# ruc-aimc-lab/GeoFormer

Hardware: AMD Instinct MI355X
Metric: image-pairs/sec (640x640) (higher is better)
Workload: dtype f16

## Files before the change

geoformer_amd/csrc/k3_linear.hip:

```cpp
#include <math.h>

#include <type_traits>

#include "gf_common.h"

#ifndef K3_TRACE
#define K3_TRACE 0
#endif
#if K3_TRACE
__device__ long long k3_trace[1024 * 4 * 16];
#define K3_T(slot) do { if (lane == 0 && blockIdx.y == 0 && blockIdx.x < 1024) k3_trace[(blockIdx.x * 4 + wave) * 16 + (slot)] = clock64(); } while (0)
extern "C" int gf_debug_k3_trace(long long* out) {
    return (int)hipMemcpyFromSymbol(out, HIP_SYMBOL(k3_trace), sizeof(long long) * 1024 * 4 * 16);
}
#else
#define K3_T(slot)
#endif

namespace {

enum { EPI_NONE = 0, EPI_RELU = 1, EPI_TANH = 2, EPI_LN = 3, EPI_LN_RES = 4, EPI_UPADD = 5 };

struct LinArgs {
    const void* a1;
    const void* a2;
    long lda1, lda2;
    int k1, k2;
    const void* w;
    const float* bias;
    const void* rgbias;
    int rg_rows;
    const float* gamma;
    const float* beta;
    float eps;
    const void* res;
    long ldres;
    const int32_t* flag;
    int flag_rows;
    void* out;
    long ldo;
    int M, N;
    const void* up_lo;
    int up_h, up_w, up_H, up_W, up_n;
    float up_ry, up_rx;
    int rm_w;
    long rm_line, rm_pix;
    const unsigned long long* rows;
    const int32_t* grp_count;
    int grp_stride, grp_rows;
};

__device__ __forceinline__ void lin_tile(int& row_tile, int& col_tile) {
    const int gx = gridDim.x, gy = gridDim.y;
    row_tile = blockIdx.x;
    col_tile = blockIdx.y;
    if (gy > 1 && (gx & 7) == 0) {
        const int id = blockIdx.y * gx + blockIdx.x, grp = id / (8 * gy), j = id - grp * (8 * gy);
        row_tile = grp * 8 + (j & 7);
        col_tile = j >> 3;
    }
}

template <typename T, int NB, int EPI, bool CONVX = false, bool AROWS = false>
__global__ __launch_bounds__(256, sizeof(T) == 2 ? 2 : 1) void linear_kernel(LinArgs a) {
    using Mm = Mma32<T>;
    using Frag = typename Mm::Frag;
    constexpr int EPC = 16 / sizeof(T);
    constexpr int BK = 128 / sizeof(T);
    constexpr int WROWS = 32 * NB;
    constexpr int ROWS = 128 + WROWS;
    constexpr int NLD = ROWS * 8 / 256;
    extern __shared__ __attribute__((aligned(16))) char smem[];
    char* st = smem;
    char* sw = smem + 128 * 128;
    float* vec = reinterpret_cast<float*>(smem + ROWS * 128);
    const int tid = threadIdx.x, lane = tid & 63, wave = tid >> 6, h = lane >> 5, lr = lane & 31;
    int row_tile, col_tile;
    lin_tile(row_tile, col_tile);
    const int m0 = row_tile * 128, n0 = col_tile * WROWS;
    const int K = a.k1 + a.k2;
    if constexpr (AROWS) {
        if (a.grp_count) {
            bool needed = false;
            const int mend = min(m0 + 128, a.M);
            for (int g = m0 / a.grp_rows, r = m0; r < mend && !needed; r = ++g * a.grp_rows)
                needed = r - g * a.grp_rows < a.grp_count[(size_t)g * a.grp_stride];
            if (!needed) return;
        }
    }

    if (tid < WROWS) {
        vec[tid] = (a.bias && n0 + tid < a.N) ? a.bias[n0 + tid] : 0.f;
        if constexpr (EPI == EPI_LN || EPI == EPI_LN_RES) {
            vec[WROWS + tid] = a.gamma[n0 + tid];
            vec[2 * WROWS + tid] = a.beta[n0 + tid];
        }
    }
    const T* src[NLD];
    int dst[NLD];
    bool isa[NLD];
#pragma unroll
    for (int p = 0; p < NLD; ++p) {
        const int e = p * 256 + tid, row = e >> 3, c = e & 7;
        isa[p] = row < 128;
        if (isa[p]) {
            src[p] = nullptr;
            if constexpr (AROWS) src[p] = reinterpret_cast<const T*>(a.rows[min(m0 + row, a.M - 1)]);
            dst[p] = gf_lds_off(row, c);
        } else {
            const int wr = row - 128;
            src[p] = (const T*)a.w + (size_t)min(n0 + wr, a.N - 1) * K + c * EPC;
            dst[p] = 128 * 128 + gf_lds_off(wr, c);
        }
    }
    v4u regs[NLD];
    const bool ragged = CONVX && (K % BK) != 0;
    auto gload = [&](int k0) {
        const bool first = k0 < a.k1;
        const T* ab = (const T*)(first ? a.a1 : a.a2);
        const long ld = first ? a.lda1 : a.lda2;
        const int kk = first ? k0 : k0 - a.k1;
#pragma unroll
        for (int p = 0; p < NLD; ++p) {
            const int e = p * 256 + tid, row = e >> 3, c = e & 7;
            const T* g;
            if (isa[p]) {
                if constexpr (AROWS) {
                    g = src[p] + k0 + c * EPC;
                } else {
                    const int r = min(m0 + row, a.M - 1);
                    const size_t ro = (CONVX && a.rm_w > 0) ? (size_t)(r / a.rm_w) * a.rm_line + (size_t)(r % a.rm_w) * a.rm_pix : (size_t)r * ld;
                    g = ab + ro + kk + c * EPC;
                }
            } else {
                g = src[p] + k0;
            }
            if constexpr (AROWS) {
                if (isa[p] && src[p] == nullptr) {
                    regs[p] = v4u{0u, 0u, 0u, 0u};
                    continue;
                }
            }
            if (!ragged || k0 + c * EPC < K) regs[p] = *reinterpret_cast<const v4u*>(g);
            else regs[p] = v4u{0u, 0u, 0u, 0u};
        }
    };
    auto lstore = [&]() {
#pragma unroll
        for (int p = 0; p < NLD; ++p) *reinterpret_cast<v4u*>(smem + dst[p]) = regs[p];
    };
    v16f acc[NB];
#pragma unroll
    for (int nb = 0; nb < NB; ++nb)
#pragma unroll
        for (int r = 0; r < 16; ++r) acc[nb][r] = 0.f;

    const int nk = (K + BK - 1) / BK;
    K3_T(0);
    gload(0);
    for (int kt = 0; kt < nk; ++kt) {
        __syncthreads();
        lstore();
        __syncthreads();
        K3_T(1 + kt);
        if (kt + 1 < nk) gload((kt + 1) * BK);
#pragma unroll
        for (int g = 0; g < 4; ++g) {
            const int chunk = 2 * g + h;
            const Frag tf = *reinterpret_cast<const Frag*>(st + gf_lds_off(wave * 32 + lr, chunk));
#pragma unroll
            for (int nb = 0; nb < NB; ++nb) {
                const Frag wf = *reinterpret_cast<const Frag*>(sw + gf_lds_off(nb * 32 + lr, chunk));
                Mm::mma(wf, tf, acc[nb]);
            }
        }
    }
    K3_T(10);
    const int token = m0 + wave * 32 + lr;
    const bool live = token < a.M;
    const int tk = live ? token : a.M - 1;
#pragma unroll
    for (int nb = 0; nb < NB; ++nb)
#pragma unroll
        for (int r = 0; r < 16; ++r) acc[nb][r] += vec[nb * 32 + gf_acc_row(r, h)];
    if (a.rgbias) {
        const T* rb = (const T*)a.rgbias + (size_t)(tk / a.rg_rows) * a.N + n0;
#pragma unroll
        for (int nb = 0; nb < NB; ++nb)
#pragma unroll
            for (int r = 0; r < 16; ++r) acc[nb][r] += gf_to_float(rb[nb * 32 + gf_acc_row(r, h)]);
    }
    if constexpr (EPI == EPI_RELU) {
#pragma unroll
        for (int nb = 0; nb < NB; ++nb)
#pragma unroll
            for (int r = 0; r < 16; ++r) acc[nb][r] = fmaxf(acc[nb][r], 0.f);
    } else if constexpr (EPI == EPI_TANH) {
#pragma unroll
        for (int nb = 0; nb < NB; ++nb)
#pragma unroll
            for (int r = 0; r < 16; ++r) {
                if constexpr (std::is_same<T, float>::value) acc[nb][r] = tanhf(acc[nb][r]);
                else acc[nb][r] = 1.0f - 2.0f * __builtin_amdgcn_rcpf(__expf(2.0f * acc[nb][r]) + 1.0f);
            }
    } else if constexpr (EPI == EPI_LN || EPI == EPI_LN_RES) {
        float s = 0.f;
#pragma unroll
        for (int nb = 0; nb < NB; ++nb)
#pragma unroll
            for (int r = 0; r < 16; ++r) s += acc[nb][r];
        s += __shfl_xor(s, 32, 64);
        const float mean = s / (float)WROWS;
        float q = 0.f;
#pragma unroll
        for (int nb = 0; nb < NB; ++nb)
#pragma unroll
            for (int r = 0; r < 16; ++r) {
                const float d = acc[nb][r] - mean;
                q += d * d;
            }
        q += __shfl_xor(q, 32, 64);
        const float rstd = 1.0f / sqrtf(q / (float)WROWS + a.eps);
#pragma unroll
        for (int nb = 0; nb < NB; ++nb)
#pragma unroll
            for (int r = 0; r < 16; ++r) {
                const int c = nb * 32 + gf_acc_row(r, h);
                acc[nb][r] = (acc[nb][r] - mean) * rstd * vec[WROWS + c] + vec[2 * WROWS + c];
            }
    }
    if constexpr (!std::is_same<T, float>::value) {
        using V4 = gf_vec<T, 4>;
        using V8 = gf_vec<T, 8>;
        constexpr int RS = 272;
        K3_T(11);
        __syncthreads();
        K3_T(12);
        char* ot = smem + wave * 32 * RS;
        const int prow = lane >> 4, pch = lane & 15;
        int upx = 0, upy = 0, upn = 0;
        if constexpr (EPI == EPI_UPADD) {
            const unsigned t0 = (unsigned)__builtin_amdgcn_readfirstlane(m0 + wave * 32);
            const unsigned q = t0 / (unsigned)a.up_W;
            upx = (int)(t0 - q * (unsigned)a.up_W);
            upy = (int)(q % (unsigned)a.up_H);
            upn = (int)(q / (unsigned)a.up_H);
        }
#pragma unroll
        for (int hb = 0; hb < (NB + 3) / 4; ++hb) {
#pragma unroll
            for (int q4 = 0; q4 < 4; ++q4)
#pragma unroll
                for (int r4 = 0; r4 < 4; ++r4) {
                    const int nb = hb * 4 + q4, c = q4 * 32 + 8 * r4 + 4 * h;
                    if (nb < NB)
                        *reinterpret_cast<V4*>(ot + lr * RS + c * 2) =
                            V4{(T)acc[nb][4 * r4], (T)acc[nb][4 * r4 + 1], (T)acc[nb][4 * r4 + 2], (T)acc[nb][4 * r4 + 3]};
                }
            __builtin_amdgcn_fence(__ATOMIC_RELEASE, "wavefront");
            __builtin_amdgcn_wave_barrier();
            __builtin_amdgcn_fence(__ATOMIC_ACQUIRE, "wavefront");
            if constexpr (EPI == EPI_UPADD) {
                const int cg = n0 + hb * 128 + pch * 8;
                const bool cok = cg < a.N;
                const T* lo = (const T*)a.up_lo + (cok ? cg : 0);
#ifdef K3_EXP_NOGATHER
#define K3_TAP(p) (*reinterpret_cast<const V8*>(lp))
#else
#define K3_TAP(p) (*reinterpret_cast<const V8*>(p))
#endif
#ifndef K3_UPADD_BATCH
#define K3_UPADD_BATCH 4
#endif
                constexpr int UB = K3_UPADD_BATCH;
#pragma unroll
                for (int b0 = 0; b0 < 8; b0 += UB) {
                V8 tap[UB][4];
                float wgt[UB][2];
#pragma unroll
                for (int ib = 0; ib < UB; ++ib) {
                    const int it = b0 + ib;
                    const int row = it * 4 + prow;
                    int px = upx + row, py = upy, pn = upn;
                    if (a.up_W >= 32) {
                        const bool wr = px >= a.up_W;
                        px -= wr ? a.up_W : 0;
                        py += wr ? 1 : 0;
                        const bool wy = py >= a.up_H;
                        py = wy ? 0 : py;
                        pn += wy ? 1 : 0;
                    } else {
                        const unsigned t = (unsigned)(m0 + wave * 32 + row), q = t / (unsigned)a.up_W;
                        px = (int)(t - q * (unsigned)a.up_W);
                        py = (int)(q % (unsigned)a.up_H);
                        pn = (int)(q / (unsigned)a.up_H);
                    }
                    pn = pn < a.up_n ? pn : a.up_n - 1;
                    const float fy = a.up_ry * py, fx = a.up_rx * px;
                    const int y0 = (int)fy, x0 = (int)fx;
                    const int y1 = y0 + (y0 < a.up_h - 1), x1 = x0 + (x0 < a.up_w - 1);
                    wgt[ib][0] = fy - y0;
                    wgt[ib][1] = fx - x0;
                    const T* lp = lo + (size_t)pn * a.up_h * a.up_w * a.N;
                    tap[ib][0] = K3_TAP(lp + ((size_t)y0 * a.up_w + x0) * a.N);
                    tap[ib][1] = K3_TAP(lp + ((size_t)y0 * a.up_w + x1) * a.N);
                    tap[ib][2] = K3_TAP(lp + ((size_t)y1 * a.up_w + x0) * a.N);
                    tap[ib][3] = K3_TAP(lp + ((size_t)y1 * a.up_w + x1) * a.N);
                }
#pragma unroll
                for (int ib = 0; ib < UB; ++ib) {
                    const int row = (b0 + ib) * 4 + prow, tg = m0 + wave * 32 + row;
                    V8 v = *reinterpret_cast<const V8*>(ot + row * RS + pch * 16);
                    const float wy1 = wgt[ib][0], wx1 = wgt[ib][1], wy0 = 1.f - wy1, wx0 = 1.f - wx1;
                    if constexpr (std::is_same<T, _Float16>::value) {
                        const float w00 = wy0 * wx0, w01 = wy0 * wx1, w10 = wy1 * wx0, w11 = wy1 * wx1;
                        const v4u uv = __builtin_bit_cast(v4u, v), u0 = __builtin_bit_cast(v4u, tap[ib][0]), u1 = __builtin_bit_cast(v4u, tap[ib][1]),
                                  u2 = __builtin_bit_cast(v4u, tap[ib][2]), u3 = __builtin_bit_cast(v4u, tap[ib][3]);
#pragma unroll
                        for (int i = 0; i < 4; ++i) {
                            float lo_, hi_;
                            asm("v_fma_mix_f32 %0, %1, %2, %3 op_sel:[0,0,0] op_sel_hi:[1,0,1]" : "=v"(lo_) : "v"(u0[i]), "v"(w00), "v"(uv[i]));
                            asm("v_fma_mix_f32 %0, %1, %2, %3 op_sel:[1,0,1] op_sel_hi:[1,0,1]" : "=v"(hi_) : "v"(u0[i]), "v"(w00), "v"(uv[i]));
                            asm("v_fma_mix_f32 %0, %1, %2, %0 op_sel:[0,0,0] op_sel_hi:[1,0,0]" : "+v"(lo_) : "v"(u1[i]), "v"(w01));
                            asm("v_fma_mix_f32 %0, %1, %2, %0 op_sel:[1,0,0] op_sel_hi:[1,0,0]" : "+v"(hi_) : "v"(u1[i]), "v"(w01));
                            asm("v_fma_mix_f32 %0, %1, %2, %0 op_sel:[0,0,0] op_sel_hi:[1,0,0]" : "+v"(lo_) : "v"(u2[i]), "v"(w10));
                            asm("v_fma_mix_f32 %0, %1, %2, %0 op_sel:[1,0,0] op_sel_hi:[1,0,0]" : "+v"(hi_) : "v"(u2[i]), "v"(w10));
                            asm("v_fma_mix_f32 %0, %1, %2, %0 op_sel:[0,0,0] op_sel_hi:[1,0,0]" : "+v"(lo_) : "v"(u3[i]), "v"(w11));
                            asm("v_fma_mix_f32 %0, %1, %2, %0 op_sel:[1,0,0] op_sel_hi:[1,0,0]" : "+v"(hi_) : "v"(u3[i]), "v"(w11));
                            v[2 * i] = (T)lo_;
                            v[2 * i + 1] = (T)hi_;
                        }
                    } else {
#pragma unroll
                        for (int i = 0; i < 8; ++i)
                            v[i] = (T)((float)v[i] + wy0 * (wx0 * (float)tap[ib][0][i] + wx1 * (float)tap[ib][1][i]) +
                                              wy1 * (wx0 * (float)tap[ib][2][i] + wx1 * (float)tap[ib][3][i]));
                    }
                    if (tg < a.M && cok) *reinterpret_cast<V8*>((T*)a.out + (size_t)tg * a.ldo + cg) = v;
                }
                }
            } else {
#pragma unroll
            for (int it = 0; it < 8; ++it) {
                const int row = it * 4 + prow, tg = m0 + wave * 32 + row, cg = n0 + hb * 128 + pch * 8;
                if (tg >= a.M || cg >= a.N) continue;
                V8 v = *reinterpret_cast<const V8*>(ot + row * RS + pch * 16);
                if constexpr (EPI == EPI_LN_RES) {
                    const V8 x = *reinterpret_cast<const V8*>((const T*)a.res + (size_t)tg * a.ldres + cg);
                    const bool keep = a.flag == nullptr || a.flag[tg / a.flag_rows] != 0;
#pragma unroll
                    for (int i = 0; i < 8; ++i) v[i] = keep ? (T)((float)x[i] + (float)v[i]) : x[i];
                }
                *reinterpret_cast<V8*>((T*)a.out + (size_t)tg * a.ldo + cg) = v;
            }
            }
            __builtin_amdgcn_fence(__ATOMIC_RELEASE, "wavefront");
            __builtin_amdgcn_wave_barrier();
            K3_T(13 + hb);
        }
    } else {
        bool keep = true;
        if constexpr (EPI == EPI_LN_RES) keep = a.flag == nullptr || a.flag[tk / a.flag_rows] != 0;
        if (!live) return;
        T* op = (T*)a.out + (size_t)token * a.ldo + n0;
        const T* rp = EPI == EPI_LN_RES ? (const T*)a.res + (size_t)token * a.ldres + n0 : nullptr;
#pragma unroll
        for (int nb = 0; nb < NB; ++nb)
#pragma unroll
            for (int r4 = 0; r4 < 4; ++r4) {
                const int c = nb * 32 + 8 * r4 + 4 * h;
                if (n0 + c >= a.N) continue;
                v4f v{acc[nb][4 * r4], acc[nb][4 * r4 + 1], acc[nb][4 * r4 + 2], acc[nb][4 * r4 + 3]};
                if constexpr (EPI == EPI_LN_RES) {
                    const v4f x = *reinterpret_cast<const v4f*>(rp + c);
                    v = keep ? v4f{x.x + v.x, x.y + v.y, x.z + v.z, x.w + v.w} : x;
                }
                *reinterpret_cast<v4f*>(op + c) = v;
            }
    }
}

template <typename T, int EPI>
__global__ __launch_bounds__(256, 2) void linear_kernel_w2(LinArgs a) {
    using Frag = typename Mma32<T>::Frag;
    using V4 = gf_vec<T, 4>;
    using V8 = gf_vec<T, 8>;
    constexpr int EPC = 8, BK = 64, WROWS = 256, ROWS = 128 + WROWS, NLD = ROWS * 8 / 256;
    extern __shared__ __attribute__((aligned(16))) char smem[];
    char* st = smem;
    char* sw = smem + 128 * 128;
    float* vec = reinterpret_cast<float*>(smem + ROWS * 128);
    const int tid = threadIdx.x, lane = tid & 63, wave = tid >> 6, h = lane >> 5, lr = lane & 31;
    const int tm = wave >> 1, tn = wave & 1;
    int row_tile, col_tile;
    lin_tile(row_tile, col_tile);
    const int m0 = row_tile * 128, n0 = col_tile * WROWS;
    const int K = a.k1 + a.k2;
    if (tid < WROWS) vec[tid] = (a.bias && n0 + tid < a.N) ? a.bias[n0 + tid] : 0.f;
    const T* src[NLD];
    int dst[NLD];
    bool isa[NLD];
#pragma unroll
    for (int p = 0; p < NLD; ++p) {
        const int e = p * 256 + tid, row = e >> 3, c = e & 7;
        isa[p] = row < 128;
        if (isa[p]) {
            src[p] = nullptr;
            dst[p] = gf_lds_off(row, c);
        } else {
            const int wr = row - 128;
            src[p] = (const T*)a.w + (size_t)min(n0 + wr, a.N - 1) * K + c * EPC;
            dst[p] = 128 * 128 + gf_lds_off(wr, c);
        }
    }
    v4u regs[NLD];
    auto gload = [&](int k0) {
        const bool first = k0 < a.k1;
        const T* ab = (const T*)(first ? a.a1 : a.a2);
        const long ld = first ? a.lda1 : a.lda2;
        const int kk = first ? k0 : k0 - a.k1;
#pragma unroll
        for (int p = 0; p < NLD; ++p) {
            const int e = p * 256 + tid, row = e >> 3, c = e & 7;
            const T* g = isa[p] ? ab + (size_t)min(m0 + row, a.M - 1) * ld + kk + c * EPC : src[p] + k0;
            regs[p] = *reinterpret_cast<const v4u*>(g);
        }
    };
    v16f acc[2][4];
#pragma unroll
    for (int t = 0; t < 2; ++t)
#pragma unroll
        for (int nb = 0; nb < 4; ++nb)
#pragma unroll
            for (int r = 0; r < 16; ++r) acc[t][nb][r] = 0.f;
    const int nk = K / BK;
    gload(0);
    for (int kt = 0; kt < nk; ++kt) {
        __syncthreads();
#pragma unroll
        for (int p = 0; p < NLD; ++p) *reinterpret_cast<v4u*>(smem + dst[p]) = regs[p];
        __syncthreads();
        if (kt + 1 < nk) gload((kt + 1) * BK);
#pragma unroll
        for (int g = 0; g < 4; ++g) {
            const int chunk = 2 * g + h;
            const Frag t0 = *reinterpret_cast<const Frag*>(st + gf_lds_off(tm * 64 + lr, chunk));
            const Frag t1 = *reinterpret_cast<const Frag*>(st + gf_lds_off(tm * 64 + 32 + lr, chunk));
#pragma unroll
            for (int nb = 0; nb < 4; ++nb) {
                const Frag wf = *reinterpret_cast<const Frag*>(sw + gf_lds_off(tn * 128 + nb * 32 + lr, chunk));
                Mma32<T>::mma(wf, t0, acc[0][nb]);
                Mma32<T>::mma(wf, t1, acc[1][nb]);
            }
        }
    }
#pragma unroll
    for (int t = 0; t < 2; ++t)
#pragma unroll
        for (int nb = 0; nb < 4; ++nb)
#pragma unroll
            for (int r = 0; r < 16; ++r) {
                float v = acc[t][nb][r] + vec[tn * 128 + nb * 32 + gf_acc_row(r, h)];
                if constexpr (EPI == EPI_RELU) v = fmaxf(v, 0.f);
                else if constexpr (EPI == EPI_TANH) v = 1.0f - 2.0f * __builtin_amdgcn_rcpf(__expf(2.0f * v) + 1.0f);
                acc[t][nb][r] = v;
            }
    constexpr int RS = 272;
    __syncthreads();
    char* ot = smem + wave * 32 * RS;
    const int prow = lane >> 4, pch = lane & 15;
#pragma unroll
    for (int t = 0; t < 2; ++t) {
#pragma unroll
        for (int nb = 0; nb < 4; ++nb)
#pragma unroll
            for (int r4 = 0; r4 < 4; ++r4) {
                const int c = nb * 32 + 8 * r4 + 4 * h;
                *reinterpret_cast<V4*>(ot + lr * RS + c * 2) =
                    V4{(T)acc[t][nb][4 * r4], (T)acc[t][nb][4 * r4 + 1], (T)acc[t][nb][4 * r4 + 2], (T)acc[t][nb][4 * r4 + 3]};
            }
        __builtin_amdgcn_fence(__ATOMIC_RELEASE, "wavefront");
        __builtin_amdgcn_wave_barrier();
        __builtin_amdgcn_fence(__ATOMIC_ACQUIRE, "wavefront");
#pragma unroll
        for (int it = 0; it < 8; ++it) {
            const int row = it * 4 + prow, tg = m0 + tm * 64 + t * 32 + row, cg = n0 + tn * 128 + pch * 8;
            if (tg >= a.M || cg >= a.N) continue;
            *reinterpret_cast<V8*>((T*)a.out + (size_t)tg * a.ldo + cg) = *reinterpret_cast<const V8*>(ot + row * RS + pch * 16);
        }
        __builtin_amdgcn_fence(__ATOMIC_RELEASE, "wavefront");
        __builtin_amdgcn_wave_barrier();
    }
}

template <typename T, int NB, int EPI, bool CONVX = false, bool AROWS = false>
void lin_launch1(const LinArgs& a, hipStream_t st) {
    constexpr int WROWS = 32 * NB;
    size_t lds = (size_t)(128 + WROWS) * 128 + 3 * WROWS * sizeof(float);
    if (lds < 4 * 32 * 272) lds = 4 * 32 * 272;
    linear_kernel<T, NB, EPI, CONVX, AROWS><<<dim3((a.M + 127) / 128, (a.N + WROWS - 1) / WROWS), 256, lds, st>>>(a);
}

template <typename T, int NB, bool AROWS = false>
void lin_launch(const LinArgs& a, int epi, hipStream_t st) {
    switch (epi) {
        case EPI_NONE: lin_launch1<T, NB, EPI_NONE, false, AROWS>(a, st); break;
        case EPI_RELU: lin_launch1<T, NB, EPI_RELU, false, AROWS>(a, st); break;
        case EPI_TANH: lin_launch1<T, NB, EPI_TANH, false, AROWS>(a, st); break;
        case EPI_LN: lin_launch1<T, NB, EPI_LN, false, AROWS>(a, st); break;
        default: lin_launch1<T, NB, EPI_LN_RES, false, AROWS>(a, st); break;
    }
}

}

extern "C" int gf_linear(const void* a1, long lda1, int k1, const void* a2, long lda2, int k2, const void* w,
                         const float* bias, const void* rowgroup_bias, int rowgroup_rows, int epilogue,
                         const float* ln_gamma, const float* ln_beta, float ln_eps, const void* residual,
                         long ldres, const int32_t* row_flag, int flag_rows, void* out, long ldo, int dtype, int M,
                         int N, void* stream) {
    GF_CHECK_ARG(a1 && w && out, "null pointer");
    GF_CHECK_ARG(M > 0 && N > 0 && k1 > 0 && k2 >= 0, "bad sizes");
    GF_CHECK_ARG(dtype >= GF_F32 && dtype <= GF_BF16, "bad dtype");
    const int bk = dtype == GF_F32 ? 32 : 64;
    GF_CHECK_ARG(k1 % bk == 0 && k2 % bk == 0, "k1 and k2 must be multiples of 32 (f32) / 64 (f16)");
    GF_CHECK_ARG(k2 == 0 || a2 != nullptr, "a2 missing");
    GF_CHECK_ARG(N % 32 == 0, "N must be a multiple of 32");
    GF_CHECK_ARG(epilogue >= EPI_NONE && epilogue <= EPI_LN_RES, "unknown epilogue");
    GF_CHECK_ARG(rowgroup_bias == nullptr || rowgroup_rows > 0, "rowgroup_rows must be > 0");
    GF_CHECK_ARG(rowgroup_bias == nullptr || N % 128 == 0, "a row-group bias needs N to be a multiple of 128 (whole column tiles)");
    const int es = dtype == GF_F32 ? 4 : 2;
    GF_CHECK_ARG((lda1 * es) % 16 == 0 && (k2 == 0 || (lda2 * es) % 16 == 0), "operand rows must be 16-byte aligned");
    GF_CHECK_ARG((ldo * es) % 16 == 0 && (uintptr_t)out % 16 == 0, "output rows must be 16-byte aligned");
    GF_CHECK_ARG(residual == nullptr || ((ldres * es) % 16 == 0 && (uintptr_t)residual % 16 == 0),
                 "residual rows must be 16-byte aligned");
    if (epilogue >= EPI_LN) {
        GF_CHECK_ARG(ln_gamma && ln_beta, "LayerNorm epilogue needs gamma and beta");
        GF_CHECK_ARG(N == 128 || N == 256, "LayerNorm epilogue is built for N = 128 or 256 (whole rows per wave pair)");
        GF_CHECK_ARG(epilogue != EPI_LN_RES || residual != nullptr, "residual missing");
        GF_CHECK_ARG(row_flag == nullptr || flag_rows > 0, "flag_rows must be > 0");
    }
    LinArgs a{a1, a2, lda1, lda2, k1, k2, w, bias, rowgroup_bias, rowgroup_rows, ln_gamma, ln_beta, ln_eps, residual,
              ldres, row_flag, flag_rows, out, ldo, M, N};
    hipStream_t st = (hipStream_t)stream;
    void* pt = gf_prof_begin("k3_linear", st, (double)es * ((double)M * (k1 + k2) + (double)N * (k1 + k2) + (double)M * N * (residual ? 2.0 : 1.0)));
    const bool wide = (epilogue >= EPI_LN) ? N == 256 : N % 256 == 0;
    if (dtype != GF_F32 && wide && epilogue <= EPI_TANH && rowgroup_bias == nullptr) {
        const size_t lds = (size_t)(128 + 256) * 128 + 256 * sizeof(float);
        const dim3 grid((M + 127) / 128, (N + 255) / 256);
#define GF_W2(T)                                                                   \
    do {                                                                           \
        if (epilogue == EPI_NONE) linear_kernel_w2<T, EPI_NONE><<<grid, 256, lds, st>>>(a);       \
        else if (epilogue == EPI_RELU) linear_kernel_w2<T, EPI_RELU><<<grid, 256, lds, st>>>(a);  \
        else linear_kernel_w2<T, EPI_TANH><<<grid, 256, lds, st>>>(a);                            \
    } while (0)
        if (dtype == GF_F16) GF_W2(_Float16);
        else GF_W2(gf_bf16);
#undef GF_W2
    } else if (dtype == GF_F32) {
        if (wide) lin_launch<float, 8>(a, epilogue, st);
        else lin_launch<float, 4>(a, epilogue, st);
    } else if (dtype == GF_F16) {
        if (wide) lin_launch<_Float16, 8>(a, epilogue, st);
        else lin_launch<_Float16, 4>(a, epilogue, st);
    } else {
        if (wide) lin_launch<gf_bf16, 8>(a, epilogue, st);
        else lin_launch<gf_bf16, 4>(a, epilogue, st);
    }
    gf_prof_end("k3_linear", pt, st);
    GF_CHECK_LAUNCH();
    return GF_OK;
}

extern "C" int gf_linear_rows(const uint64_t* row_table, int row_align, const int32_t* group_count, int group_count_stride, int group_rows,
                              int k, const void* w, const float* bias, const void* rowgroup_bias, int rowgroup_rows, int epilogue,
                              const float* ln_gamma, const float* ln_beta, float ln_eps, const void* residual, long ldres,
                              const int32_t* row_flag, int flag_rows, void* out, long ldo, int dtype, int M, int N, void* stream) {
    GF_CHECK_ARG(row_table && w && out, "null pointer");
    GF_CHECK_ARG(dtype == GF_F16 || dtype == GF_BF16, "built for the 16-bit types (fp32: gf_linear on a gathered copy)");
    GF_CHECK_ARG(M > 0 && N > 0 && k > 0, "bad sizes");
    GF_CHECK_ARG(k % 64 == 0, "k must be a multiple of 64");
    GF_CHECK_ARG(N % 32 == 0, "N must be a multiple of 32");
    GF_CHECK_ARG(epilogue >= EPI_NONE && epilogue <= EPI_LN_RES, "unknown epilogue");
    GF_CHECK_ARG(rowgroup_bias == nullptr || rowgroup_rows > 0, "rowgroup_rows must be > 0");
    GF_CHECK_ARG(rowgroup_bias == nullptr || N % 128 == 0, "a row-group bias needs N to be a multiple of 128 (whole column tiles)");
    GF_CHECK_ARG(row_align > 0 && (row_align & (row_align - 1)) == 0 && row_align % 16 == 0, "operand rows must be 16-byte aligned (row_align: a power of two >= 16)");
    GF_CHECK_ARG((uintptr_t)row_table % 8 == 0, "the row table must be 8-byte aligned");
    GF_CHECK_ARG(group_count == nullptr || (group_rows > 0 && group_count_stride >= 0), "group_rows must be > 0");
    GF_CHECK_ARG((ldo * 2) % 16 == 0 && (uintptr_t)out % 16 == 0, "output rows must be 16-byte aligned");
    GF_CHECK_ARG(residual == nullptr || ((ldres * 2) % 16 == 0 && (uintptr_t)residual % 16 == 0), "residual rows must be 16-byte aligned");
    if (epilogue >= EPI_LN) {
        GF_CHECK_ARG(ln_gamma && ln_beta, "LayerNorm epilogue needs gamma and beta");
        GF_CHECK_ARG(N == 128 || N == 256, "LayerNorm epilogue is built for N = 128 or 256 (whole rows per wave pair)");
        GF_CHECK_ARG(epilogue != EPI_LN_RES || residual != nullptr, "residual missing");
        GF_CHECK_ARG(row_flag == nullptr || flag_rows > 0, "flag_rows must be > 0");
    }
    LinArgs a{nullptr, nullptr, 0, 0, k, 0, w, bias, rowgroup_bias, rowgroup_rows, ln_gamma, ln_beta, ln_eps, residual,
              ldres, row_flag, flag_rows, out, ldo, M, N};
    a.rows = (const unsigned long long*)row_table;
    a.grp_count = group_count; a.grp_stride = group_count_stride; a.grp_rows = group_rows;
    hipStream_t st = (hipStream_t)stream;
    const double rows_moved = group_count ? 0.0 : (double)M;
    void* pt = gf_prof_begin("k3_linear", st, 2.0 * (rows_moved * k + (double)N * k + rows_moved * N * (residual ? 2.0 : 1.0)) + 8.0 * M);
    const bool wide = (epilogue >= EPI_LN) ? N == 256 : N % 256 == 0;
    if (dtype == GF_F16) {
        if (wide) lin_launch<_Float16, 8, true>(a, epilogue, st);
        else lin_launch<_Float16, 4, true>(a, epilogue, st);
    } else {
        if (wide) lin_launch<gf_bf16, 8, true>(a, epilogue, st);
        else lin_launch<gf_bf16, 4, true>(a, epilogue, st);
    }
    gf_prof_end("k3_linear", pt, st);
    GF_CHECK_LAUNCH();
    return GF_OK;
}

namespace {
__global__ __launch_bounds__(256) void index_rows_kernel(const char* x, long row_bytes, const int32_t* idx, long idx_stride, int N, int L,
                                                         unsigned long long* rows) {
    const long e = (long)blockIdx.x * 256 + threadIdx.x;
    if (e >= (long)N * L) return;
    const long n = e / L, j = e - n * L;
    const int t = min(max(idx[n * idx_stride + j], 0), L - 1);
    rows[e] = (unsigned long long)(uintptr_t)(x + (n * L + t) * row_bytes);
}
}

extern "C" int gf_index_rows(const void* x, long row_bytes, const int32_t* idx, long idx_stride, int N, int L, uint64_t* rows, void* stream) {
    GF_CHECK_ARG(x && idx && rows, "null pointer");
    GF_CHECK_ARG(N > 0 && L > 0 && (long)N * L < (1l << 31) && row_bytes > 0 && idx_stride >= 0, "bad sizes");
    index_rows_kernel<<<(unsigned)(((long)N * L + 255) / 256), 256, 0, (hipStream_t)stream>>>((const char*)x, row_bytes, idx, idx_stride, N, L,
                                                                                              (unsigned long long*)rows);
    GF_CHECK_LAUNCH();
    return GF_OK;
}

extern "C" int gf_conv1x1_upsample_add_nhwc(const void* x, const void* w, const void* lo, void* out, int N, int h, int wl,
                                            int H, int W, int Cin, int Cout, int dtype, void* stream) {
    GF_CHECK_ARG(x && w && lo && out, "null pointer");
    GF_CHECK_ARG(N > 0 && h > 0 && wl > 0 && H > 0 && W > 0, "empty problem");
    GF_CHECK_ARG(dtype == GF_F16 || dtype == GF_BF16, "built for 16-bit maps (the inference backbone)");
    GF_CHECK_ARG(Cin % 32 == 0 && Cout % 32 == 0, "Cin and Cout must be multiples of 32");
    GF_CHECK_ARG((long)N * H * W < (1l << 31), "too many pixels");
    GF_CHECK_ARG((uintptr_t)x % 16 == 0 && (uintptr_t)out % 16 == 0 && (uintptr_t)lo % 16 == 0, "tensors must be 16-byte aligned");
    LinArgs a{};
    a.a1 = x; a.lda1 = Cin; a.k1 = Cin; a.w = w; a.out = out; a.ldo = Cout; a.M = N * H * W; a.N = Cout;
    a.up_lo = lo; a.up_h = h; a.up_w = wl; a.up_H = H; a.up_W = W; a.up_n = N;
    a.up_ry = H > 1 ? (float)(h - 1) / (float)(H - 1) : 0.f;
    a.up_rx = W > 1 ? (float)(wl - 1) / (float)(W - 1) : 0.f;
    hipStream_t st = (hipStream_t)stream;
    void* pt = gf_prof_begin("k3_upadd", st, 2.0 * ((double)a.M * (Cin + Cout) + (double)N * h * wl * Cout + (double)Cin * Cout));
    if (dtype == GF_F16) lin_launch1<_Float16, 4, EPI_UPADD, true>(a, st);
    else lin_launch1<gf_bf16, 4, EPI_UPADD, true>(a, st);
    gf_prof_end("k3_upadd", pt, st);
    GF_CHECK_LAUNCH();
    return GF_OK;
}

extern "C" int gf_conv1x1_nhwc(const void* x, const void* w, void* out, int N, int H, int W, int Cin, int Cout, int stride, int dtype,
                               void* stream) {
    GF_CHECK_ARG(x && w && out, "null pointer");
    GF_CHECK_ARG(N > 0 && H > 0 && W > 0, "empty problem");
    GF_CHECK_ARG(stride == 1 || (stride == 2 && H % 2 == 0 && W % 2 == 0), "stride 1, or 2 on even-sized maps");
    GF_CHECK_ARG(dtype == GF_F16 || dtype == GF_BF16, "built for 16-bit maps (the inference backbone)");
    GF_CHECK_ARG(Cin % 32 == 0 && Cout % 32 == 0, "Cin and Cout must be multiples of 32");
    GF_CHECK_ARG((long)N * H * W < (1l << 31), "too many pixels");
    GF_CHECK_ARG((uintptr_t)x % 16 == 0 && (uintptr_t)out % 16 == 0 && (uintptr_t)w % 16 == 0, "tensors must be 16-byte aligned");
    const int oh = H / stride, ow = W / stride;
    LinArgs a{};
    a.a1 = x; a.lda1 = Cin; a.k1 = Cin; a.w = w; a.out = out; a.ldo = Cout; a.M = N * oh * ow; a.N = Cout;
    if (stride == 2) { a.rm_w = ow; a.rm_line = 2l * W * Cin; a.rm_pix = 2l * Cin; }
    hipStream_t st = (hipStream_t)stream;
    void* pt = gf_prof_begin("conv1x1", st, 2.0 * ((double)a.M * (Cin + Cout) + (double)Cin * Cout));
    if (dtype == GF_F16) lin_launch1<_Float16, 4, EPI_NONE, true>(a, st);
    else lin_launch1<gf_bf16, 4, EPI_NONE, true>(a, st);
    gf_prof_end("conv1x1", pt, st);
    GF_CHECK_LAUNCH();
    return GF_OK;
}
```

Measured before the change: 731.2.

## Add persistent streaming GEMM for small-K linears with register-resident weights

Adds a persistent linear_stream kernel for K<=256 that keeps each wave's weight fragment in registers and double-buffers 64-row activation tiles into LDS by DMA. Each block loops over tiles assigned per XCD, so the next tile's load overlaps the current tile's MMA and epilogue. The kernel is routed ahead of the existing paths for linear, conv1x1 and upsample-add calls, and the bilinear blend is factored into a shared helper. In exchange it adds a new code path with 32-bit offset limits and an XCD-based tile split whose load balance and occupancy may differ from the tiled kernels.

```diff
diff --git a/geoformer_amd/csrc/k3_linear.hip b/geoformer_amd/csrc/k3_linear.hip
--- a/geoformer_amd/csrc/k3_linear.hip
+++ b/geoformer_amd/csrc/k3_linear.hip
@@ -58,6 +58,35 @@
         const int id = blockIdx.y * gx + blockIdx.x, grp = id / (8 * gy), j = id - grp * (8 * gy);
         row_tile = grp * 8 + (j & 7);
         col_tile = j >> 3;
+    }
+}
+
+template <typename T>
+__device__ __forceinline__ void k3_upadd_blend(gf_vec<T, 8>& v, const gf_vec<T, 8> (&tap)[4], float wy1, float wx1) {
+    const float wy0 = 1.f - wy1, wx0 = 1.f - wx1;
+    if constexpr (std::is_same<T, _Float16>::value) {
+        const float w00 = wy0 * wx0, w01 = wy0 * wx1, w10 = wy1 * wx0, w11 = wy1 * wx1;
+        const v4u uv = __builtin_bit_cast(v4u, v), u0 = __builtin_bit_cast(v4u, tap[0]), u1 = __builtin_bit_cast(v4u, tap[1]),
+                  u2 = __builtin_bit_cast(v4u, tap[2]), u3 = __builtin_bit_cast(v4u, tap[3]);
+#pragma unroll
+        for (int i = 0; i < 4; ++i) {
+            float lo_, hi_;
+            asm("v_fma_mix_f32 %0, %1, %2, %3 op_sel:[0,0,0] op_sel_hi:[1,0,1]" : "=v"(lo_) : "v"(u0[i]), "v"(w00), "v"(uv[i]));
+            asm("v_fma_mix_f32 %0, %1, %2, %3 op_sel:[1,0,1] op_sel_hi:[1,0,1]" : "=v"(hi_) : "v"(u0[i]), "v"(w00), "v"(uv[i]));
+            asm("v_fma_mix_f32 %0, %1, %2, %0 op_sel:[0,0,0] op_sel_hi:[1,0,0]" : "+v"(lo_) : "v"(u1[i]), "v"(w01));
+            asm("v_fma_mix_f32 %0, %1, %2, %0 op_sel:[1,0,0] op_sel_hi:[1,0,0]" : "+v"(hi_) : "v"(u1[i]), "v"(w01));
+            asm("v_fma_mix_f32 %0, %1, %2, %0 op_sel:[0,0,0] op_sel_hi:[1,0,0]" : "+v"(lo_) : "v"(u2[i]), "v"(w10));
+            asm("v_fma_mix_f32 %0, %1, %2, %0 op_sel:[1,0,0] op_sel_hi:[1,0,0]" : "+v"(hi_) : "v"(u2[i]), "v"(w10));
+            asm("v_fma_mix_f32 %0, %1, %2, %0 op_sel:[0,0,0] op_sel_hi:[1,0,0]" : "+v"(lo_) : "v"(u3[i]), "v"(w11));
+            asm("v_fma_mix_f32 %0, %1, %2, %0 op_sel:[1,0,0] op_sel_hi:[1,0,0]" : "+v"(hi_) : "v"(u3[i]), "v"(w11));
+            v[2 * i] = (T)lo_;
+            v[2 * i + 1] = (T)hi_;
+        }
+    } else {
+#pragma unroll
+        for (int i = 0; i < 8; ++i)
+            v[i] = (T)((float)v[i] + wy0 * (wx0 * (float)tap[0][i] + wx1 * (float)tap[1][i]) +
+                       wy1 * (wx0 * (float)tap[2][i] + wx1 * (float)tap[3][i]));
     }
 }
 
@@ -311,31 +340,7 @@
                 for (int ib = 0; ib < UB; ++ib) {
                     const int row = (b0 + ib) * 4 + prow, tg = m0 + wave * 32 + row;
                     V8 v = *reinterpret_cast<const V8*>(ot + row * RS + pch * 16);
-                    const float wy1 = wgt[ib][0], wx1 = wgt[ib][1], wy0 = 1.f - wy1, wx0 = 1.f - wx1;
-                    if constexpr (std::is_same<T, _Float16>::value) {
-                        const float w00 = wy0 * wx0, w01 = wy0 * wx1, w10 = wy1 * wx0, w11 = wy1 * wx1;
-                        const v4u uv = __builtin_bit_cast(v4u, v), u0 = __builtin_bit_cast(v4u, tap[ib][0]), u1 = __builtin_bit_cast(v4u, tap[ib][1]),
-                                  u2 = __builtin_bit_cast(v4u, tap[ib][2]), u3 = __builtin_bit_cast(v4u, tap[ib][3]);
-#pragma unroll
-                        for (int i = 0; i < 4; ++i) {
-                            float lo_, hi_;
-                            asm("v_fma_mix_f32 %0, %1, %2, %3 op_sel:[0,0,0] op_sel_hi:[1,0,1]" : "=v"(lo_) : "v"(u0[i]), "v"(w00), "v"(uv[i]));
-                            asm("v_fma_mix_f32 %0, %1, %2, %3 op_sel:[1,0,1] op_sel_hi:[1,0,1]" : "=v"(hi_) : "v"(u0[i]), "v"(w00), "v"(uv[i]));
-                            asm("v_fma_mix_f32 %0, %1, %2, %0 op_sel:[0,0,0] op_sel_hi:[1,0,0]" : "+v"(lo_) : "v"(u1[i]), "v"(w01));
-                            asm("v_fma_mix_f32 %0, %1, %2, %0 op_sel:[1,0,0] op_sel_hi:[1,0,0]" : "+v"(hi_) : "v"(u1[i]), "v"(w01));
-                            asm("v_fma_mix_f32 %0, %1, %2, %0 op_sel:[0,0,0] op_sel_hi:[1,0,0]" : "+v"(lo_) : "v"(u2[i]), "v"(w10));
-                            asm("v_fma_mix_f32 %0, %1, %2, %0 op_sel:[1,0,0] op_sel_hi:[1,0,0]" : "+v"(hi_) : "v"(u2[i]), "v"(w10));
-                            asm("v_fma_mix_f32 %0, %1, %2, %0 op_sel:[0,0,0] op_sel_hi:[1,0,0]" : "+v"(lo_) : "v"(u3[i]), "v"(w11));
-                            asm("v_fma_mix_f32 %0, %1, %2, %0 op_sel:[1,0,0] op_sel_hi:[1,0,0]" : "+v"(hi_) : "v"(u3[i]), "v"(w11));
-                            v[2 * i] = (T)lo_;
-                            v[2 * i + 1] = (T)hi_;
-                        }
-                    } else {
-#pragma unroll
-                        for (int i = 0; i < 8; ++i)
-                            v[i] = (T)((float)v[i] + wy0 * (wx0 * (float)tap[ib][0][i] + wx1 * (float)tap[ib][1][i]) +
-                                              wy1 * (wx0 * (float)tap[ib][2][i] + wx1 * (float)tap[ib][3][i]));
-                    }
+                    k3_upadd_blend<T>(v, tap[ib], wgt[ib][0], wgt[ib][1]);
                     if (tg < a.M && cok) *reinterpret_cast<V8*>((T*)a.out + (size_t)tg * a.ldo + cg) = v;
                 }
                 }
@@ -491,6 +496,197 @@
         __builtin_amdgcn_fence(__ATOMIC_RELEASE, "wavefront");
         __builtin_amdgcn_wave_barrier();
     }
+}
+
+constexpr int ST_TM = 64;
+constexpr int ST_OT = ST_TM * 256;
+
+template <typename T, int KG, int EPI>
+__global__ __launch_bounds__(256, 2) void linear_stream(LinArgs a, int tiles, int ncb, unsigned a_bytes) {
+    using Mm = Mma32<T>;
+    using Frag = typename Mm::Frag;
+    using V4 = gf_vec<T, 4>;
+    using V8 = gf_vec<T, 8>;
+    constexpr int RB = KG * 32, CPR = RB / 16, RPP = 64 / CPR, NP = ST_TM / RPP / 4, TILE = ST_TM * RB;
+    extern __shared__ __attribute__((aligned(16))) char smem[];
+    char* ot = smem + 2 * TILE;
+    const int tid = threadIdx.x, lane = tid & 63, wave = __builtin_amdgcn_readfirstlane(tid >> 6), h = lane >> 5, lr = lane & 31;
+    const int xcd = blockIdx.x & 7, slot = blockIdx.x >> 3, per_xcd = gridDim.x >> 3;
+    const int cb = slot % ncb, rl = slot / ncb, nrl = per_xcd / ncb;
+    const int tq = tiles >> 3, trem = tiles & 7;
+    const int tbeg = xcd < trem ? xcd * (tq + 1) : trem * (tq + 1) + (xcd - trem) * tq, tcnt = tq + (xcd < trem ? 1 : 0);
+    if (rl >= tcnt) return;
+    const int K = a.k1, n0 = cb * 128, nw = n0 + wave * 32;
+    Frag af[KG];
+    {
+        const T* wp = (const T*)a.w + (size_t)min(nw + lr, a.N - 1) * K + h * 8;
+#pragma unroll
+        for (int kg = 0; kg < KG; ++kg) {
+            if (kg * 16 < K) af[kg] = *reinterpret_cast<const Frag*>(wp + kg * 16);
+            else af[kg] = __builtin_bit_cast(Frag, v4u{0u, 0u, 0u, 0u});
+        }
+    }
+    float bv[16];
+#pragma unroll
+    for (int r = 0; r < 16; ++r) {
+        const int n = nw + gf_acc_row(r, h);
+        bv[r] = (a.bias && n < a.N) ? a.bias[n] : 0.f;
+    }
+    const GfRsrc ars = gf_rsrc(a.a1, a_bytes);
+    auto dma = [&](int tile, int buf) {
+        int dl = lane;
+        asm volatile("" : "+v"(dl));
+#pragma unroll
+        for (int i = 0; i < NP; ++i) {
+            const int p = wave * NP + i, row = p * RPP + dl / CPR, c = (dl % CPR) ^ (row & 15);
+            const unsigned r = (unsigned)(tile * ST_TM + row);
+            unsigned ro;
+            if (a.rm_w > 0) {
+                const unsigned y = r / (unsigned)a.rm_w;
+                ro = y * (unsigned)a.rm_line + (r - y * (unsigned)a.rm_w) * (unsigned)a.rm_pix;
+            } else {
+                ro = r * (unsigned)a.lda1;
+            }
+            const bool in = r < (unsigned)a.M && c * 8 < K;
+            gf_lds_dma(ars, smem + buf * TILE + p * 1024, in ? (int)((ro + c * 8) * (unsigned)sizeof(T)) : 0x7FFFFFF0, 0);
+        }
+    };
+    dma(tbeg + rl, 0);
+    int it = 0;
+    for (int ti = rl; ti < tcnt; ti += nrl, ++it) {
+        const int tile = tbeg + ti, m0 = tile * ST_TM;
+        asm volatile("s_waitcnt vmcnt(0)" ::: "memory");
+        __syncthreads();
+        if (ti + nrl < tcnt) dma(tile + nrl, (it + 1) & 1);
+        const char* tb = smem + (it & 1) * TILE;
+        v16f acc[2];
+#pragma unroll
+        for (int t = 0; t < 2; ++t)
+#pragma unroll
+            for (int r = 0; r < 16; ++r) acc[t][r] = 0.f;
+#pragma unroll
+        for (int kg = 0; kg < KG; ++kg) {
+            const int chunk = 2 * kg + h;
+            const Frag b0 = *reinterpret_cast<const Frag*>(tb + lr * RB + ((chunk ^ (lr & 15)) << 4));
+            const Frag b1 = *reinterpret_cast<const Frag*>(tb + (32 + lr) * RB + ((chunk ^ (lr & 15)) << 4));
+            Mm::mma(af[kg], b0, acc[0]);
+            Mm::mma(af[kg], b1, acc[1]);
+        }
+#pragma unroll
+        for (int t = 0; t < 2; ++t)
+#pragma unroll
+            for (int r = 0; r < 16; ++r) acc[t][r] += bv[r];
+        if (a.rgbias) {
+#pragma unroll
+            for (int t = 0; t < 2; ++t) {
+                const int tk = min(m0 + t * 32 + lr, a.M - 1);
+                const T* rb = (const T*)a.rgbias + (size_t)(tk / a.rg_rows) * a.N + nw;
+#pragma unroll
+                for (int r = 0; r < 16; ++r) acc[t][r] += gf_to_float(rb[gf_acc_row(r, h)]);
+            }
+        }
+        if constexpr (EPI == EPI_RELU) {
+#pragma unroll
+            for (int t = 0; t < 2; ++t)
+#pragma unroll
+                for (int r = 0; r < 16; ++r) acc[t][r] = fmaxf(acc[t][r], 0.f);
+        } else if constexpr (EPI == EPI_TANH) {
+#pragma unroll
+            for (int t = 0; t < 2; ++t)
+#pragma unroll
+                for (int r = 0; r < 16; ++r) acc[t][r] = 1.0f - 2.0f * __builtin_amdgcn_rcpf(__expf(2.0f * acc[t][r]) + 1.0f);
+        }
+#pragma unroll
+        for (int t = 0; t < 2; ++t)
+#pragma unroll
+            for (int r4 = 0; r4 < 4; ++r4) {
+                const int row = t * 32 + lr, chunk = wave * 4 + r4;
+                *reinterpret_cast<V4*>(ot + row * 256 + ((chunk ^ (row & 15)) << 4) + h * 8) =
+                    V4{(T)acc[t][4 * r4], (T)acc[t][4 * r4 + 1], (T)acc[t][4 * r4 + 2], (T)acc[t][4 * r4 + 3]};
+            }
+        __syncthreads();
+        const int prow = tid >> 4, pch = tid & 15, cg = n0 + pch * 8;
+        const bool cok = cg < a.N;
+        if constexpr (EPI == EPI_UPADD) {
+            const T* lo = (const T*)a.up_lo + (cok ? cg : 0);
+            V8 tap[4][4];
+            float wgt[4][2];
+#pragma unroll
+            for (int ib = 0; ib < 4; ++ib) {
+                const unsigned tg = (unsigned)(m0 + ib * 16 + prow), q = tg / (unsigned)a.up_W;
+                const int px = (int)(tg - q * (unsigned)a.up_W), py = (int)(q % (unsigned)a.up_H);
+                int pn = (int)(q / (unsigned)a.up_H);
+                pn = pn < a.up_n ? pn : a.up_n - 1;
+                float fy = a.up_ry * py, fx = a.up_rx * px;
+                asm volatile("" : "+v"(fy), "+v"(fx));
+                const int y0 = (int)fy, x0 = (int)fx;
+                const int y1 = y0 + (y0 < a.up_h - 1), x1 = x0 + (x0 < a.up_w - 1);
+                wgt[ib][0] = fy - y0;
+                wgt[ib][1] = fx - x0;
+                const T* lp = lo + (size_t)pn * a.up_h * a.up_w * a.N;
+                tap[ib][0] = *reinterpret_cast<const V8*>(lp + ((size_t)y0 * a.up_w + x0) * a.N);
+                tap[ib][1] = *reinterpret_cast<const V8*>(lp + ((size_t)y0 * a.up_w + x1) * a.N);
+                tap[ib][2] = *reinterpret_cast<const V8*>(lp + ((size_t)y1 * a.up_w + x0) * a.N);
+                tap[ib][3] = *reinterpret_cast<const V8*>(lp + ((size_t)y1 * a.up_w + x1) * a.N);
+            }
+#pragma unroll
+            for (int ib = 0; ib < 4; ++ib) {
+                const int row = ib * 16 + prow, tg = m0 + row;
+                V8 v = *reinterpret_cast<const V8*>(ot + row * 256 + ((pch ^ (row & 15)) << 4));
+                k3_upadd_blend<T>(v, tap[ib], wgt[ib][0], wgt[ib][1]);
+                if (tg < a.M && cok) *reinterpret_cast<V8*>((T*)a.out + (size_t)tg * a.ldo + cg) = v;
+            }
+        } else {
+#pragma unroll
+            for (int ib = 0; ib < 4; ++ib) {
+                const int row = ib * 16 + prow, tg = m0 + row;
+                if (tg < a.M && cok)
+                    *reinterpret_cast<V8*>((T*)a.out + (size_t)tg * a.ldo + cg) = *reinterpret_cast<const V8*>(ot + row * 256 + ((pch ^ (row & 15)) << 4));
+            }
+        }
+    }
+}
+
+template <typename T, int KG>
+void lin_stream_launch(const LinArgs& a, int epi, int tiles, int ncb, int grid, unsigned a_bytes, hipStream_t st) {
+    constexpr int LDS = 2 * ST_TM * KG * 32 + ST_OT;
+    static std::atomic<uint64_t> attr{0};
+    if (LDS > 64 * 1024 && gf_first_use_on_device(attr)) {
+        (void)hipFuncSetAttribute((const void*)linear_stream<T, KG, EPI_NONE>, hipFuncAttributeMaxDynamicSharedMemorySize, LDS);
+        (void)hipFuncSetAttribute((const void*)linear_stream<T, KG, EPI_RELU>, hipFuncAttributeMaxDynamicSharedMemorySize, LDS);
+        (void)hipFuncSetAttribute((const void*)linear_stream<T, KG, EPI_TANH>, hipFuncAttributeMaxDynamicSharedMemorySize, LDS);
+        if constexpr (std::is_same<T, _Float16>::value)
+            (void)hipFuncSetAttribute((const void*)linear_stream<T, KG, EPI_UPADD>, hipFuncAttributeMaxDynamicSharedMemorySize, LDS);
+    }
+    switch (epi) {
+        case EPI_NONE: linear_stream<T, KG, EPI_NONE><<<grid, 256, LDS, st>>>(a, tiles, ncb, a_bytes); break;
+        case EPI_RELU: linear_stream<T, KG, EPI_RELU><<<grid, 256, LDS, st>>>(a, tiles, ncb, a_bytes); break;
+        case EPI_TANH: linear_stream<T, KG, EPI_TANH><<<grid, 256, LDS, st>>>(a, tiles, ncb, a_bytes); break;
+        default:
+            if constexpr (std::is_same<T, _Float16>::value) linear_stream<T, KG, EPI_UPADD><<<grid, 256, LDS, st>>>(a, tiles, ncb, a_bytes);
+            break;
+    }
+}
+
+bool lin_stream(const LinArgs& a, int epi, int dtype, hipStream_t st) {
+    const int K = a.k1;
+    if (dtype == GF_F32 || a.k2 != 0 || a.rows != nullptr || K % 16 != 0 || K > 256 || a.N > 64 * 128) return false;
+    if (epi != EPI_NONE && epi != EPI_RELU && epi != EPI_TANH && epi != EPI_UPADD) return false;
+    if (epi == EPI_UPADD && dtype != GF_F16) return false;
+    const long last = a.M - 1;
+    const double span = 2.0 * ((a.rm_w > 0 ? (double)(last / a.rm_w) * a.rm_line + (double)(last % a.rm_w) * a.rm_pix : (double)last * a.lda1) + K);
+    if (span >= (double)0x7FFFFFF0) return false;
+    if (a.rm_w > 0 && (a.rm_line < 0 || a.rm_pix < 0)) return false;
+    const int tiles = (a.M + ST_TM - 1) / ST_TM, ncb = (a.N + 127) / 128, per = (tiles + 7) / 8;
+    const int nrl = per < 64 / ncb ? per : 64 / ncb, grid = 8 * nrl * ncb;
+    if (dtype == GF_F16) {
+        if (K <= 128) lin_stream_launch<_Float16, 8>(a, epi, tiles, ncb, grid, (unsigned)span, st);
+        else lin_stream_launch<_Float16, 16>(a, epi, tiles, ncb, grid, (unsigned)span, st);
+    } else {
+        if (K <= 128) lin_stream_launch<gf_bf16, 8>(a, epi, tiles, ncb, grid, (unsigned)span, st);
+        else lin_stream_launch<gf_bf16, 16>(a, epi, tiles, ncb, grid, (unsigned)span, st);
+    }
+    return true;
 }
 
 template <typename T, int NB, int EPI, bool CONVX = false, bool AROWS = false>
@@ -545,7 +741,8 @@
     hipStream_t st = (hipStream_t)stream;
     void* pt = gf_prof_begin("k3_linear", st, (double)es * ((double)M * (k1 + k2) + (double)N * (k1 + k2) + (double)M * N * (residual ? 2.0 : 1.0)));
     const bool wide = (epilogue >= EPI_LN) ? N == 256 : N % 256 == 0;
-    if (dtype != GF_F32 && wide && epilogue <= EPI_TANH && rowgroup_bias == nullptr) {
+    if (lin_stream(a, epilogue, dtype, st)) {
+    } else if (dtype != GF_F32 && wide && epilogue <= EPI_TANH && rowgroup_bias == nullptr) {
         const size_t lds = (size_t)(128 + 256) * 128 + 256 * sizeof(float);
         const dim3 grid((M + 127) / 128, (N + 255) / 256);
 #define GF_W2(T)                                                                   \
@@ -650,7 +847,8 @@
     a.up_rx = W > 1 ? (float)(wl - 1) / (float)(W - 1) : 0.f;
     hipStream_t st = (hipStream_t)stream;
     void* pt = gf_prof_begin("k3_upadd", st, 2.0 * ((double)a.M * (Cin + Cout) + (double)N * h * wl * Cout + (double)Cin * Cout));
-    if (dtype == GF_F16) lin_launch1<_Float16, 4, EPI_UPADD, true>(a, st);
+    if (lin_stream(a, EPI_UPADD, dtype, st)) {
+    } else if (dtype == GF_F16) lin_launch1<_Float16, 4, EPI_UPADD, true>(a, st);
     else lin_launch1<gf_bf16, 4, EPI_UPADD, true>(a, st);
     gf_prof_end("k3_upadd", pt, st);
     GF_CHECK_LAUNCH();
@@ -672,7 +870,8 @@
     if (stride == 2) { a.rm_w = ow; a.rm_line = 2l * W * Cin; a.rm_pix = 2l * Cin; }
     hipStream_t st = (hipStream_t)stream;
     void* pt = gf_prof_begin("conv1x1", st, 2.0 * ((double)a.M * (Cin + Cout) + (double)Cin * Cout));
-    if (dtype == GF_F16) lin_launch1<_Float16, 4, EPI_NONE, true>(a, st);
+    if (lin_stream(a, EPI_NONE, dtype, st)) {
+    } else if (dtype == GF_F16) lin_launch1<_Float16, 4, EPI_NONE, true>(a, st);
     else lin_launch1<gf_bf16, 4, EPI_NONE, true>(a, st);
     gf_prof_end("conv1x1", pt, st);
     GF_CHECK_LAUNCH();
```

Measured after the change: 720.9. -1.4%, worse.
